# bcgsc/btl_bloomfilter

Hardware: AMD Instinct MI355X
Metric: Mk-mers/s insert+query, k=31 h=4, 64 GiB filter (higher is better)
Workload: dtype u64

## Files before the change

btl_bloomfilter_amd/build.py:

```python
import os
import subprocess
import sys
from concurrent.futures import ThreadPoolExecutor

HERE = os.path.dirname(os.path.abspath(__file__))
CSRC = os.path.join(HERE, "csrc")
TAG = os.environ.get("BTLBF_BUILD_TAG", "")
OBJ = os.path.join(HERE, "_build" + ("_" + TAG if TAG else ""))
LIB = os.path.join(HERE, "libbtlbf%s.so" % ("_" + TAG if TAG else ""))
HEADERS = ["internal.hpp", "mibf_plan.hpp", "mibf_zip.hpp", "mibf_classify_core.hpp", "host_internal.hpp", "host_partition.hpp", "device_utils.hpp", "seq_core.hpp", "partition_core.hpp",
           os.path.join("..", "..", "include", "btlbf.h")]
HOST_UNITS = ["capi", "host_io", "host_seq", "host_query", "host_partition", "host_aux", "host_mibf", "host_mibf_probs",
              "host_mibf_fastx", "fastx"]
KERNEL_UNITS = ["seq_kernels", "aux_kernels", "split_query_kernels", "partition_kernels", "mibf_kernels", "mibf_classify_kernels",
                "mibf_classify_pair_kernels", "mibf_stream_kernels"]
UNITS = [(u, u + ".cpp", []) for u in HOST_UNITS] + [(u, u + ".hip", []) for u in KERNEL_UNITS]
UNITS += [("part_hash_h%d" % h, "part_hash_inst.hip", ["-DBTLBF_PART_H=%d" % h]) for h in range(1, 9)]
FLAGS = ["--offload-arch=gfx950", "-O3", "-std=c++17", "-fPIC", "-Wall", "-Wno-unused-function"]


def _newest_header():
    return max(os.path.getmtime(os.path.join(CSRC, h)) for h in HEADERS + ["../build.py"])


def _extra_flags():
# ... 51 lines not shown
```

btl_bloomfilter_amd/csrc/host_partition.cpp:

```cpp
#include "../../include/btlbf.h"
#include "internal.hpp"
#include "host_internal.hpp"
#include "host_partition.hpp"

#include <algorithm>
#include <cmath>
#include <cstdlib>
#include <cstring>
#include <vector>

using namespace btlbf;

namespace {

static constexpr uint64_t kFailCap = 4ull << 20;
static constexpr uint64_t kFailTableSlots = 2 * kFailCap;
static constexpr uint64_t kFreshSpillCap = 16ull << 20;

uint32_t chunks_for(double mean_entries, uint32_t tail_chunks, uint32_t epc = kChunk)
{
	const double m = mean_entries + 8.0 * std::sqrt(mean_entries + 1.0) + 32.0;
	return (uint32_t)std::min<double>(4.0e9, std::ceil(m / (double)epc)) + tail_chunks;
}

unsigned ceil_log2(uint64_t x)
{
	unsigned b = 0;
	while ((1ull << b) < x)
		++b;
	return b;
}

bool plan_segments(uint64_t mloc, PartPlan& pl, uint32_t unit_shift = 3)
{
	const uint32_t small = 16 + unit_shift;
	pl.counting = unit_shift == 0;
	pl.seg_shift = small;
	if (((mloc + (1ull << small) - 1) >> small) > 512ull * 1024)
// ... 56 lines not shown
		for (int j = 1; j < pl.n_levels; ++j) {
			pl.lv[j].regions = split_slices(bins_g, r_in, cus);
			r_in = pl.lv[j].regions;
			bins_g *= pl.lv[j].P;
		}
	}
	return true;
}

bool packed_enabled()
{
	const char* e = getenv("BTLBF_PACKED");
	return !(e && e[0] == '0');
}

void plan_caps(PartPlan& pl, double entries, int first_level)
{
	pl.bytes_total = 0;
	for (int j = first_level; j < pl.n_levels; ++j) {
		PartLevel& l = pl.lv[j];
		const double useful = j == pl.n_levels - 1 ? (double)std::min<uint64_t>(pl.n_seg, l.bins) : (double)l.bins;
		l.packed = j >= 1 && j == pl.n_levels - 1 && !pl.counting && part_packs(l.P, l.shift) && packed_enabled();
		l.cap = chunks_for(entries / (useful * l.regions), 1, part_epc(l.packed));
		l.alloc_bins = l.bins;
		if (j >= 1 && pl.group_bins) {
			l.alloc_bins = pl.group_bins;
			for (int i = 1; i <= j; ++i)
				l.alloc_bins *= pl.lv[i].P;
		}
		l.cnt_bytes = ((uint64_t)l.alloc_bins * l.regions * 4 + 255) / 256 * 256;
		l.ent_bytes = (uint64_t)l.alloc_bins * l.regions * l.cap * (kChunk * 4);
		pl.bytes_total += l.cnt_bytes + l.ent_bytes;
	}
}

uint8_t* carve_levels(PartPlan& pl, uint8_t* p, int first_level)
{
	for (int j = first_level; j < pl.n_levels; ++j) {
		pl.lv[j].cnt = reinterpret_cast<uint32_t*>(p);
		p += pl.lv[j].cnt_bytes;
		pl.lv[j].ent = reinterpret_cast<uint32_t*>(p);
		p += pl.lv[j].ent_bytes;
	}
	return p;
}

unsigned cu_count(int device)
{
	int cus = 256;
	(void)hipDeviceGetAttribute(&cus, hipDeviceAttributeMultiprocessorCount, device);
	return (unsigned)cus;
}

uint64_t tiles_for_caps(uint64_t tiles, uint32_t regions)
{
	return regions ? (tiles + regions - 1) / regions * regions : tiles;
}

double probes_per_tile(const btlbf_filter* f, const PartTiling& tl)
{
	return tl.windows_per_tile * f->hp.h + 1.0;
}

PartSide part_side(const btlbf_filter* f, const PartPlan* pl = nullptr)
{
	PartSide sd;
	memset(&sd, 0, sizeof sd);
	sd.pos_base = f->mod.shard_lo;
	sd.counting = f->kind == BTLBF_COUNTING8;
	sd.threshold = f->thr;
	if (pl) {
		sd.late_buf = pl->late_buf;
		sd.late_cap = pl->late_cap;
		sd.bin_wseg = pl->lv[0].wseg;
		sd.bin_magic = pl->lv[0].wseg ? (uint32_t)(((1ull << 32) + pl->lv[0].wseg - 1) / pl->lv[0].wseg) : 0;
		sd.bin_seg_shift = pl->seg_shift;
		sd.bin_width = pl->lv[0].wseg << pl->seg_shift;
	}
	return sd;
}

int run_levels(btlbf_filter* f, PartPlan& pl, PartIn in0, const PartSide& sd, int query, hipStream_t s,
               uint32_t bin_offset = 0, uint32_t n_bins0 = 0)
{
	const int exact = sd.counting && !query;
	if (f->lazy_zero && !(sd.fresh && !query))
		return fail(BTLBF_EINVAL, "internal error: partition passes on a lazily cleared array");
	const int prof_split = query ? BTLBF_PROF_QUERY_SPLIT : BTLBF_PROF_INSERT_SPLIT;
	const int prof_apply = query ? BTLBF_PROF_QUERY_TEST : BTLBF_PROF_INSERT_APPLY;
	if (n_bins0 == 0)
		n_bins0 = pl.lv[0].bins - bin_offset;
	const uint32_t group = pl.group(n_bins0);
	for (uint32_t b0 = 0; b0 < n_bins0; b0 += group) {
		PartIn in = in0;
		uint32_t first_in = b0, abs_first = bin_offset + b0, n_in = std::min(group, n_bins0 - b0);
		uint32_t in_shift = pl.lv[0].shift;
		for (int j = 1; j < pl.n_levels; ++j) {
			ProfSpan ps(f, prof_split, s);
			HIP_TRY(launch_part_split(f->d_data, in, first_in, abs_first, n_in, pl.lv[j].out(), pl.lv[j].shift,
			                          in_shift, sd, query, exact, s));
			in = pl.lv[j].in();
			first_in = 0;
			abs_first *= pl.lv[j].P;
			n_in *= pl.lv[j].P;
			in_shift = pl.lv[j].shift;
		}
		const uint64_t seg_first = abs_first;
		if (seg_first >= pl.n_seg)
			break;
		const uint64_t n_seg = std::min<uint64_t>(n_in, pl.n_seg - seg_first);
		ProfSpan ps(f, prof_apply, s);
		HIP_TRY(launch_part_apply(f->d_data, f->local_bytes, pl.seg_shift, seg_first, n_seg, in, sd, query, s));
	}
	return BTLBF_OK;
}

constexpr double kAutoInsertRatio = 0.0095;
constexpr double kWideSplitProbes = 1.6e10;

}

namespace btlbf {

PartTail part_tail(uint64_t budget)
{
	PartTail t;
	const bool full = budget >= (2ull << 30);
// ... 88 lines not shown
	if (level0)
		pl = *level0;
	else if (!plan_level0(f, pl, call_probes(f, base.len)))
		return pp;
	PartLevel& l0 = pl.lv[0];
	l0.regions = cu_count(f->device);
	if (!plan_splits(pl, l0.regions, cu_count(f->device)) || !part_hash_fits(f->hp, l0.P))
		return pp;
	pp.tiling = part_tiling(f->hp, l0.P, base.layout, base.len);
	const uint64_t budget = scratch_budget(f);
	pp.tail = part_tail(budget);
	pl.late_cap = budget >= (2ull << 30) ? part_late_cap() : 0;
	const uint64_t late_bytes = (uint64_t)l0.regions * 2 * pl.late_cap * sizeof(uint32_t);
	const uint64_t extra_bytes = ((pp.tail.bytes + 255) / 256) * 256 + late_bytes;
	const double ppt = probes_per_tile(f, pp.tiling) * ((double)f->mod.shard_len / (double)f->mod.size);
	uint64_t tiles = pp.tiling.n_tiles;
	for (int iter = 0; iter < 64; ++iter) {
		plan_caps(pl, (double)tiles_for_caps(tiles, l0.regions) * ppt, 0);
		pl.bytes_total += extra_bytes;
		if (pl.bytes_total <= budget || tiles <= 1)
			break;
		const double ratio = (double)budget / (double)pl.bytes_total;
		const uint64_t nt = (uint64_t)((double)tiles * ratio * 0.95);
		tiles = nt >= tiles ? tiles - 1 : (nt ? nt : 1);
	}
	if (pl.bytes_total > budget)
		return pp;
	if (mode == BTLBF_INSERT_AUTO && tiles < pp.tiling.n_tiles && (double)tiles * ppt < auto_ratio * (double)f->local_bytes)
		return pp;
	pl.tiles_per_batch = tiles;
	if (!f->part.grow(pl.bytes_total, f->device))
		return pp;
	pp.extra = carve_levels(pl, static_cast<uint8_t*>(f->part.p), 0);
	pl.late_buf = pl.late_cap ? reinterpret_cast<uint32_t*>(pp.extra + ((pp.tail.bytes + 255) / 256) * 256) : nullptr;
	pp.ok = true;
	return pp;
}

struct RoutePlan {
	uint32_t n_windows = 1;
	uint32_t shards_per_window = 1;
	uint32_t window_shift = 0;
	uint32_t bins = 1024;
	uint32_t shift0 = 0;
	uint32_t bins_per_shard = 0;
	uint32_t regions = 0;
	uint32_t cap = 0;
	uint64_t ent_bytes_per_shard = 0, cnt_bytes_per_shard = 0;
// ... 23 lines not shown
	rp.bins = rp.window_shift - 9 <= 32 && rp.shards_per_window <= 512 ? 512 : 1024;
	if (const char* e = getenv("BTLBF_ROUTE_BINS")) {
		const unsigned b = (unsigned)atoi(e);
		if (b >= rp.shards_per_window && b <= 1024 && !(b & (b - 1)))
			rp.bins = b;
	}
	const unsigned lw = rp.window_shift, lb = ceil_log2(rp.bins);
	const unsigned seg_min = f->kind == BTLBF_COUNTING8 ? 16 : 19;
	if (lw < lb + seg_min || lw - lb > 32 || rp.bins < rp.shards_per_window)
		return fail(BTLBF_EINVAL, "routing supports global filters of at least 2^29 bits (2^26 counters)");
	rp.shift0 = lw - lb;
	rp.bins_per_shard = rp.bins / rp.shards_per_window;
	rp.regions = cu_count(f->device);
	const PartTiling tl = part_tiling(f->hp, rp.bins, lay, len);
	const double entries = (double)tiles_for_caps(tl.n_tiles, rp.regions) * probes_per_tile(f, tl) / rp.n_windows;
	rp.cap = chunks_for(entries / ((double)rp.bins * rp.regions), 1);
	rp.ent_bytes_per_shard = (uint64_t)rp.bins_per_shard * rp.regions * rp.cap * (kChunk * 4);
	rp.cnt_bytes_per_shard = (uint64_t)rp.bins_per_shard * rp.regions * 4;
	return BTLBF_OK;
}

int owner_plan(btlbf_filter* f, const RoutePlan& rp, const LayoutParams& lay, uint64_t plan_len, unsigned n_blocks,
               unsigned n_shards, PartPlan& pl)
{
	if (!plan_segments(f->mod.shard_len, pl, f->kind == BTLBF_COUNTING8 ? 0 : 3))
		return fail(BTLBF_EINVAL, "shard too large for the partitioned pipeline");
	pl.lv[0].bins = rp.bins_per_shard;
	pl.lv[0].shift = rp.shift0;
	pl.lv[0].regions = rp.regions * n_blocks;
	if (pl.lv[0].shift < pl.seg_shift || !plan_splits(pl, pl.lv[0].regions, cu_count(f->device)))
		return fail(BTLBF_EINVAL, "unsupported shard geometry");
// ... 69 lines not shown
		return false;
	if (f->insert_mode == BTLBF_INSERT_PARTITIONED)
		return true;
	return worth_sweep(f, local_probes(f, len), kAutoInsertRatio);
}

int partitioned_insert(btlbf_filter* f, const SeqArgs& base, hipStream_t s, bool* done)
{
	*done = false;
	PartPrep pp = part_prepare(f, base, f->insert_mode, kAutoInsertRatio);
	if (!pp.ok)
		return BTLBF_OK;
	PartPlan& pl = pp.pl;
	const uint64_t total_tiles = pp.tiling.n_tiles;
	for (uint64_t t0 = 0; t0 < total_tiles; t0 += pl.tiles_per_batch) {
		SeqArgs a = base;
		a.first_tile = t0;
		a.n_tiles = std::min<uint64_t>(pl.tiles_per_batch, total_tiles - t0);
		for (int attempt = 0; attempt < 2; ++attempt) {
			const bool fresh = f->lazy_zero;
			PartSide sd = part_side(f, &pl);
			if (fresh) {
				HIP_TRY(order_after_clear(f, s));
				sd.fresh = 1;
				sd.spill_count = reinterpret_cast<unsigned long long*>(pp.extra);
				sd.spill_list = reinterpret_cast<uint64_t*>(pp.extra + 256);
				sd.spill_cap = pp.tail.spill_cap;
				HIP_TRY(hipMemsetAsync(sd.spill_count, 0, 8, s));
			}
			{
				ProfSpan ps(f, BTLBF_PROF_INSERT_HASH, s);
				HIP_TRY(launch_part_hash(a, pl.lv[0].out(), pl.lv[0].shift, sd, 0, s));
			}
			if (int rc = run_levels(f, pl, pl.lv[0].in(), sd, 0, s))
				return rc;
			if (!fresh)
				break;
			f->lazy_zero = false;
			unsigned long long n_spill = 0;
			hipError_t e = hipMemcpyAsync(&n_spill, sd.spill_count, 8, hipMemcpyDeviceToHost, s);
			if (e == hipSuccess)
				e = hipStreamSynchronize(s);
			if (e == hipSuccess && n_spill <= pp.tail.spill_cap) {
				e = launch_spill(f->d_data, sd.spill_list, n_spill, f->mod.shard_lo, f->mod.shard_len, 0, part_side(f), s);
				if (e == hipSuccess)
					break;
			}
			if (e != hipSuccess) {
				f->lazy_zero = true;
// ... 15 lines not shown
		return BTLBF_OK;
	PartPlan& pl = pp.pl;
	const uint64_t total_tiles = pp.tiling.n_tiles;
	PartSide sd = part_side(f, &pl);
	sd.fail_count = reinterpret_cast<unsigned long long*>(pp.extra);
	sd.fail_list = reinterpret_cast<uint64_t*>(pp.extra + 256);
	sd.fail_cap = pp.tail.fail_cap;
	const int direct_op = direct_query_op(f);
	uint64_t* table = sd.fail_list + pp.tail.fail_cap;
	uint64_t* ctl = reinterpret_cast<uint64_t*>(pp.extra + 64);
	if (counts)
		HIP_TRY(hipMemsetAsync(counts, 0, 16, s));
	const uint64_t seq_tw = (uint64_t)seq_tile_windows();
	const uint64_t seq_tiles_all = (base.len + seq_tw - 1) / seq_tw;
	for (uint64_t t0 = 0; t0 < total_tiles; t0 += pl.tiles_per_batch) {
		SeqArgs a = base;
		a.first_tile = t0;
		a.n_tiles = std::min<uint64_t>(pl.tiles_per_batch, total_tiles - t0);
		a.hit_bits = hit_bits;
		a.valid_bits = valid_bits;
		a.counts = counts;
		HIP_TRY(hipMemsetAsync(sd.fail_count, 0, 8, s));
		{
			ProfSpan ps(f, BTLBF_PROF_QUERY_HASH, s);
			HIP_TRY(launch_part_hash(a, pl.lv[0].out(), pl.lv[0].shift, sd, 1, s));
		}
		if (int rc = run_levels(f, pl, pl.lv[0].in(), sd, 1, s))
			return rc;
		const uint64_t first = t0 * pp.tiling.tile_bytes / seq_tw;
		const uint64_t end_b = std::min<uint64_t>(base.len, (t0 + a.n_tiles) * (uint64_t)pp.tiling.tile_bytes);
		const uint64_t n = std::min<uint64_t>((end_b + seq_tw - 1) / seq_tw, seq_tiles_all) - first;
		ProfSpan ps(f, BTLBF_PROF_QUERY_RESOLVE, s);
		HIP_TRY(launch_failset_auto(sd.fail_list, sd.fail_count, pp.tail.fail_cap, table, pp.tail.table_slots, ctl, s));
		SeqArgs d = base;
		d.first_tile = first;
		d.n_tiles = n;
		d.hit_bits = hit_bits;
		d.valid_bits = nullptr;
		d.counts = nullptr;
		d.gate = ctl;
		d.gate_mode = GATE_REDO;
		REQUIRE_MATERIALIZED(f);
		HIP_TRY(launch_seq_op(direct_op, d, s));
		d.buckets = table;
		d.gate_mode = GATE_RESOLVE;
// ... 204 lines not shown
```

btl_bloomfilter_amd/csrc/host_partition.hpp:

```cpp
#pragma once
#include "host_internal.hpp"

namespace btlbf {

struct PartTail {
	uint64_t fail_cap, table_slots, spill_cap, bytes;
};
PartTail part_tail(uint64_t budget);

struct PartLevel {
	uint32_t bins = 0;
	uint32_t P = 0;
	uint32_t regions = 0;
	uint32_t cap = 0;
	uint32_t shift = 0;
	uint32_t wseg = 0;
	uint32_t alloc_bins = 0;
	uint32_t packed = 0;
	uint64_t cnt_bytes = 0, ent_bytes = 0;
	uint32_t* cnt = nullptr;
	uint32_t* ent = nullptr;
	PartOut out() const { return PartOut{P, regions, cap, packed, cnt, ent}; }
	PartIn in() const { return PartIn{1, alloc_bins, regions, cap, cnt, ent, packed}; }
};

struct PartPlan {
	uint32_t seg_shift = 19;
	uint64_t n_seg = 0;
	bool counting = false;
	uint32_t group_bins = 0;
	int n_levels = 0;
	PartLevel lv[3];
	uint64_t tiles_per_batch = 0;
	uint64_t bytes_total = 0;
	uint32_t* late_buf = nullptr;
	uint32_t late_cap = 0;
	uint32_t group(uint32_t n_bins0) const { return n_levels >= 2 && group_bins ? group_bins : n_bins0; }
};

constexpr double kAutoQueryRatio = 0.0165;

uint64_t scratch_budget(btlbf_filter* f);
double local_probes(const btlbf_filter* f, uint64_t len);
bool worth_sweep(const btlbf_filter* f, double probes, double ratio);
int direct_query_op(const btlbf_filter* f);
double call_probes(const btlbf_filter* f, uint64_t len);
bool plan_level0(const btlbf_filter* f, PartPlan& pl, double call_probes = 0);

int part_query(btlbf_filter* f, const SeqArgs& base, uint8_t* hit_bits, uint8_t* valid_bits, uint64_t* counts,
               hipStream_t s, bool* done, bool defer_hit_count, const PartPlan* level0);

// ... 2 lines not shown
```

btl_bloomfilter_amd/csrc/internal.hpp:

```cpp
#pragma once
#include <hip/hip_runtime.h>
#include <stdint.h>

#include "mibf_plan.hpp"

namespace btlbf {

static constexpr uint64_t kSeedA = 0x3c8bfbb395c60474ULL;
static constexpr uint64_t kSeedC = 0x3193c18562a02b4cULL;
static constexpr uint64_t kSeedG = 0x20323ed082572324ULL;
static constexpr uint64_t kSeedT = 0x295549f54be24456ULL;
static constexpr uint64_t kMultiSeed = 0x90b45d39fb6da1faULL;
static constexpr unsigned kMultiShift = 27;

static constexpr unsigned kCodeShift = 4u;
static constexpr unsigned kCodeOff = 0x70u;
static constexpr unsigned kNumCodes = 8u;
static constexpr unsigned kBaseValid = 1u;
static constexpr unsigned kBaseGood = 2u;

static constexpr uint32_t kChunk = 32;
static constexpr uint32_t kChunkShift = 5;
static constexpr uint32_t kPackChunk = 48;
static constexpr uint32_t kPackBits = 20;
// ... 140 lines not shown
	uint32_t late_cap;
	uint32_t* late_buf;
	uint32_t bin_wseg, bin_magic, bin_seg_shift, bin_width;
};
static inline uint32_t part_late_cap() { return 32768u; }

PartTiling part_tiling(const HashParams& hp, uint32_t p0, const LayoutParams& lay, uint64_t len);
bool part_supported(const HashParams& hp);
bool part_hash_fits(const HashParams& hp, uint32_t p0);
hipError_t launch_part_hash(const SeqArgs& a, const PartOut& out, uint32_t bin_shift, const PartSide& sd, int query,
                            hipStream_t s);
hipError_t launch_part_split(void* filter, const PartIn& in, uint32_t first_in, uint32_t abs_first, uint32_t n_in_bins,
                             const PartOut& out, uint32_t sub_shift, uint32_t in_shift, const PartSide& sd, int query,
                             int exact, hipStream_t s);
hipError_t launch_part_apply(void* filter, uint64_t local_bytes, uint32_t seg_shift, uint64_t seg_first, uint64_t n_seg,
                             const PartIn& in, const PartSide& sd, int query, hipStream_t s);
hipError_t launch_failset_build(const uint64_t* fail_list, uint64_t n, uint64_t* table, uint64_t mask, hipStream_t s);
enum { GATE_NONE = 0, GATE_RESOLVE = 1, GATE_REDO = 2 };
hipError_t launch_failset_auto(const uint64_t* fail_list, const unsigned long long* fail_count, uint64_t fail_cap,
                               uint64_t* table, uint64_t max_slots, uint64_t* ctl, hipStream_t s);
hipError_t launch_spill(void* filter, const uint64_t* pos, uint64_t n, uint64_t lo, uint64_t len, int test,
                        const PartSide& sd, hipStream_t s);
hipError_t launch_seq_op(int op, const SeqArgs& a, hipStream_t s);
hipError_t launch_hash_op(int op, void* filter, const ModParams& mod, uint32_t h, uint32_t threshold,
                          const uint64_t* hashes, uint64_t n, uint8_t* out, int serial, hipStream_t s,
                          const uint8_t* row_valid = nullptr);
hipError_t launch_kmer_rows(const uint8_t* kmers, uint64_t n, uint32_t k, uint32_t h, uint64_t kms, uint64_t* rows,
                            uint8_t* valid, hipStream_t s);
hipError_t launch_serial_seq_update(const SeqArgs& a, int op, const uint64_t* hashes,
                                    const uint8_t* valid_bits, uint8_t* out, hipStream_t s);
hipError_t launch_popcount(const void* data, uint64_t nbytes, int mode, uint32_t threshold,
// ... 123 lines not shown
```

btl_bloomfilter_amd/csrc/partition_kernels.hip:

```cpp
#include "partition_core.hpp"
#include <algorithm>

namespace btlbf {

typedef uint32_t v4u_t __attribute__((ext_vector_type(4)));
__device__ __forceinline__ uint4 nt_load4(const uint4* p)
{
	const v4u_t v = __builtin_nontemporal_load(reinterpret_cast<const v4u_t*>(p));
	return make_uint4(v.x, v.y, v.z, v.w);
}
__device__ __forceinline__ void nt_store4(uint4* p, const uint4& q)
{
	v4u_t v = {q.x, q.y, q.z, q.w};
	__builtin_nontemporal_store(v, reinterpret_cast<v4u_t*>(p));
}

__device__ __forceinline__ uint32_t part_in_region(const PartIn& in, uint32_t b, uint32_t r)
{
	return ((r / in.regions_per_block) * in.bins_per_block + b) * in.regions_per_block + r % in.regions_per_block;
}

template <bool QUERY, bool EXACT, bool PK>
__global__ __launch_bounds__(kPartThreads) void part_split_kernel(void* filter, const PartIn in, const PartOut out,
                                                                 const uint32_t slices, const uint32_t sub_shift,
// ... 73 lines not shown
			if (base1 >= n_vec)
				break;
			if (base1 + kPartThreads * kVec < n_vec)
				fetch(va, base1 + kPartThreads * kVec);
			round(vb, base1);
		}
	}
	if (PK)
		part_finish_pk<kPartThreads>(pl, out, bin0, g, ovf);
	else
		part_finish<kPartThreads>(pl, out, bin0, g, ovf);
}

static constexpr uint32_t kApplyMaxRegions = 1024;
static constexpr uint32_t kApplyFewRegions = 16;

enum ApplyMode : int {
	APPLY_BIT_OR = 0,
	APPLY_BIT_TEST = 1,
	APPLY_CNT_INC = 2,
	APPLY_CNT_TEST = 3
};

template <int MODE>
__device__ __forceinline__ void apply_entry(uint32_t* lds, uint32_t e, const PartSide& sd, uint64_t seg_base)
{
	if (MODE == APPLY_BIT_OR) {
		atomicOr(&lds[e >> 5], 1u << (e & 31));
	} else if (MODE == APPLY_BIT_TEST) {
		if (!((lds[e >> 5] >> (e & 31)) & 1u))
// ... 42 lines not shown
	} else {
		if (left > 0)
			apply_entry<MODE>(lds, q.x, sd, seg_base);
		if (left > 1)
			apply_entry<MODE>(lds, q.y, sd, seg_base);
		if (left > 2)
			apply_entry<MODE>(lds, q.z, sd, seg_base);
		if (left > 3)
			apply_entry<MODE>(lds, q.w, sd, seg_base);
	}
}

template <int MODE, int NT, bool PK>
__global__ __launch_bounds__(NT) void part_apply_kernel(uint8_t* filter, uint64_t local_bytes,
                                                        uint32_t seg_shift, uint32_t seg_first,
                                                        const PartIn in, const PartSide sd)
{
	constexpr bool QUERY = (MODE & 1) != 0;
	constexpr bool kNtEnt = !QUERY;
	constexpr uint32_t kUnitShift = MODE >= APPLY_CNT_INC ? 0 : 3;
	extern __shared__ __attribute__((aligned(16))) uint8_t dyn[];
	__shared__ uint32_t any;
	__shared__ uint32_t r_n[kApplyMaxRegions];
	__shared__ uint32_t r_reg[kApplyMaxRegions];
	const uint32_t tid = threadIdx.x;
	const uint32_t ibin = blockIdx.x;
	const uint32_t seg = seg_first + blockIdx.x;
	const uint32_t n_regions = in.blocks * in.regions_per_block;
	constexpr uint32_t kVecE = PK ? 6 : 4;
	const uint32_t cap_entries = in.cap * (PK ? kPackChunk : kChunk);
	const uint32_t cap_words = in.cap * kChunk;
	const bool tabled = n_regions <= kApplyMaxRegions;
	if (tid == 0)
		any = 0;
	__syncthreads();
	uint32_t mine = 0;
	for (uint32_t r = tid; r < n_regions; r += NT) {
		const uint32_t reg = part_in_region(in, ibin, r);
		uint32_t n = in.cnt[reg];
		if (n > cap_entries)
			n = cap_entries;
		mine |= n;
		if (tabled) {
			r_n[r] = n;
			r_reg[r] = reg;
		}
	}
	if (mine)
		any = 1;
	__syncthreads();
	if (!any && !(sd.fresh && !QUERY))
		return;
	const uint64_t seg_bytes = 1ull << (seg_shift - kUnitShift);
	const uint64_t byte0 = (uint64_t)seg * seg_bytes;
	const uint64_t seg_base = (uint64_t)seg << seg_shift;
	uint64_t nbytes = local_bytes - byte0;
	if (nbytes > seg_bytes)
		nbytes = seg_bytes;
	const uint32_t n_vec = (uint32_t)((nbytes + 15) / 16);
	uint4* lds4 = reinterpret_cast<uint4*>(dyn);
// ... 4 lines not shown
	uint4 q[kEntU];
#define BTLBF_SETTLE(r, i)                               \
	while ((r) < n_regions) {                            \
		const uint32_t nev__ = (r_n[(r)] + kVecE - 1) / kVecE; \
		if ((i) < nev__)                                 \
			break;                                       \
		(i) -= nev__;                                    \
		++(r);                                           \
	}
#define BTLBF_FETCH(dst, lft, u)                                                                               \
	do {                                                                                                       \
		lft = 0;                                                                                               \
		dst = make_uint4(0, 0, 0, 0);                                                                          \
		if (wr[u] < n_regions) {                                                                               \
			lft = r_n[wr[u]] - wi[u] * kVecE;                                                                  \
			dst = reinterpret_cast<const uint4*>(in.ent + (uint64_t)r_reg[wr[u]] * cap_words)[wi[u]];          \
		}                                                                                                      \
	} while (0)
	constexpr int kFewU = 3;
	const bool few = tabled && n_regions <= kApplyFewRegions;
	uint4 fq[kFewU];
	uint32_t fl[kFewU];
	uint32_t f_r = 0, f_off = 0;
	auto few_nvec = [&](uint32_t r) -> uint32_t {
		return ((uint32_t)__builtin_amdgcn_readfirstlane((int)r_n[r]) + kVecE - 1) / kVecE;
	};
	auto few_skip = [&]() {
		while (f_r < n_regions && f_off >= few_nvec(f_r)) {
			++f_r;
			f_off = 0;
		}
	};
	auto few_request = [&](uint4 (&d)[kFewU], uint32_t (&lf)[kFewU]) {
		const uint32_t n0 = (uint32_t)__builtin_amdgcn_readfirstlane((int)r_n[f_r]), nv0 = (n0 + kVecE - 1) / kVecE;
		const uint32_t reg0 = (uint32_t)__builtin_amdgcn_readfirstlane((int)r_reg[f_r]);
		const bool two = f_r + 1 < n_regions;
		const uint32_t n1 = two ? (uint32_t)__builtin_amdgcn_readfirstlane((int)r_n[two ? f_r + 1 : f_r]) : 0u, nv1 = (n1 + kVecE - 1) / kVecE;
		const uint32_t reg1 = two ? (uint32_t)__builtin_amdgcn_readfirstlane((int)r_reg[two ? f_r + 1 : f_r]) : reg0;
		const uint4* src0 = reinterpret_cast<const uint4*>(in.ent + (uint64_t)reg0 * cap_words);
		const uint4* src1 = reinterpret_cast<const uint4*>(in.ent + (uint64_t)reg1 * cap_words);
#pragma unroll
		for (int u = 0; u < kFewU; ++u) {
			const uint32_t v = f_off + (uint32_t)u * NT + tid;
			lf[u] = 0;
			d[u] = make_uint4(0, 0, 0, 0);
			if (v < nv0) {
				d[u] = kNtEnt ? nt_load4(src0 + v) : src0[v];
				lf[u] = n0 - v * kVecE;
			} else if (v - nv0 < nv1) {
				d[u] = kNtEnt ? nt_load4(src1 + (v - nv0)) : src1[v - nv0];
				lf[u] = n1 - (v - nv0) * kVecE;
			}
		}
		const uint32_t end = f_off + (uint32_t)(kFewU * NT);
		if (end <= nv0) {
// ... 67 lines not shown
				wi[u] += kEntU * NT;
				BTLBF_SETTLE(wr[u], wi[u])
				BTLBF_FETCH(nq[u], nleft[u], u);
			}
#pragma unroll
			for (int u = 0; u < kEntU; ++u) {
				apply_vec<MODE, PK>(lds, q[u], left[u], sd, seg_base);
				q[u] = nq[u];
				left[u] = nleft[u];
			}
		}
#undef BTLBF_SETTLE
#undef BTLBF_FETCH
	} else {
		for (uint32_t r = 0; r < n_regions; ++r) {
			const uint32_t reg = part_in_region(in, ibin, r);
			uint32_t n = in.cnt[reg];
			if (n > cap_entries)
				n = cap_entries;
			const uint32_t* e1 = in.ent + (uint64_t)reg * cap_words;
			if (PK) {
				for (uint32_t i = tid; i < (n + 2) / 3; i += NT) {
					uint32_t e3[3];
					part_unpack3(e1[2 * i], e1[2 * i + 1], e3);
					apply_entry<MODE>(lds, e3[0], sd, seg_base);
					apply_entry<MODE>(lds, e3[1], sd, seg_base);
					apply_entry<MODE>(lds, e3[2], sd, seg_base);
				}
				continue;
			}
			for (uint32_t i = tid; i < n; i += NT)
				apply_entry<MODE>(lds, e1[i], sd, seg_base);
		}
	}
	if (QUERY)
// ... 168 lines not shown
	                   abs_first - first_in, sd);
}

template <int NT>
static auto apply_kernel(int mode, bool packed) -> decltype(&part_apply_kernel<APPLY_BIT_OR, NT, false>)
{
	switch (mode) {
	case APPLY_BIT_OR: return packed ? &part_apply_kernel<APPLY_BIT_OR, NT, true> : &part_apply_kernel<APPLY_BIT_OR, NT, false>;
	case APPLY_BIT_TEST: return packed ? &part_apply_kernel<APPLY_BIT_TEST, NT, true> : &part_apply_kernel<APPLY_BIT_TEST, NT, false>;
	case APPLY_CNT_INC: return &part_apply_kernel<APPLY_CNT_INC, NT, false>;
	default: return &part_apply_kernel<APPLY_CNT_TEST, NT, false>;
	}
}

hipError_t launch_part_apply(void* filter, uint64_t local_bytes, uint32_t seg_shift, uint64_t seg_first, uint64_t n_seg,
                             const PartIn& in, const PartSide& sd, int query, hipStream_t s)
{
	if (n_seg == 0)
		return hipSuccess;
	if (in.packed && (sd.counting || seg_shift > kPackBits))
		return hipErrorInvalidValue;
	const int mode = (sd.counting ? APPLY_CNT_INC : APPLY_BIT_OR) + (query ? 1 : 0);
	const size_t dyn = (size_t)1 << (seg_shift - (sd.counting ? 0 : 3));
	const bool wide = dyn > 64 * 1024;
	return part_launch(wide ? apply_kernel<1024>(mode, in.packed) : apply_kernel<512>(mode, in.packed), dim3((unsigned)n_seg),
	                   dim3(wide ? 1024 : 512), dyn, s, static_cast<uint8_t*>(filter), local_bytes, seg_shift, (uint32_t)seg_first,
	                   in, sd);
}

__device__ __forceinline__ void failset_insert(unsigned long long* table, uint64_t mask, unsigned long long key)
{
	uint64_t slot = mix64(key) & mask;
	for (;;) {
		const unsigned long long prev = atomicCAS(&table[slot], 0ull, key);
		if (prev == 0ull || prev == key)
			break;
		slot = (slot + 1) & mask;
	}
}
__global__ __launch_bounds__(256) void failset_build_kernel(const uint64_t* list, uint64_t n,
                                                           unsigned long long* table, uint64_t mask)
{
// ... 90 lines not shown
```

Baseline: 61730.

## Carry level-0 split batches into a single final apply pass over the filter

When the partition scratch budget forces the input to be split into several tile batches, earlier batches are now hashed and split into per-batch carried buckets instead of each running a full apply pass. The final batch's apply kernel then reads both the current and carried buckets, so each filter segment is loaded into LDS and written back once per call instead of once per batch. A planner in a new header picks the number of carried batches and their sizes to fit the budget. The cost is more scratch bookkeeping, extra split launches, and an apply kernel that addresses regions through a shared arena base with 32-bit chunk offsets.

```diff
diff --git a/btl_bloomfilter_amd/build.py b/btl_bloomfilter_amd/build.py
--- a/btl_bloomfilter_amd/build.py
+++ b/btl_bloomfilter_amd/build.py
@@ -8,7 +8,7 @@
 TAG = os.environ.get("BTLBF_BUILD_TAG", "")
 OBJ = os.path.join(HERE, "_build" + ("_" + TAG if TAG else ""))
 LIB = os.path.join(HERE, "libbtlbf%s.so" % ("_" + TAG if TAG else ""))
-HEADERS = ["internal.hpp", "mibf_plan.hpp", "mibf_zip.hpp", "mibf_classify_core.hpp", "host_internal.hpp", "host_partition.hpp", "device_utils.hpp", "seq_core.hpp", "partition_core.hpp",
+HEADERS = ["internal.hpp", "mibf_plan.hpp", "part_plan.hpp", "mibf_zip.hpp", "mibf_classify_core.hpp", "host_internal.hpp", "host_partition.hpp", "device_utils.hpp", "seq_core.hpp", "partition_core.hpp",
            os.path.join("..", "..", "include", "btlbf.h")]
 HOST_UNITS = ["capi", "host_io", "host_seq", "host_query", "host_partition", "host_aux", "host_mibf", "host_mibf_probs",
               "host_mibf_fastx", "fastx"]
diff --git a/btl_bloomfilter_amd/csrc/host_partition.cpp b/btl_bloomfilter_amd/csrc/host_partition.cpp
--- a/btl_bloomfilter_amd/csrc/host_partition.cpp
+++ b/btl_bloomfilter_amd/csrc/host_partition.cpp
@@ -2,9 +2,11 @@
 #include "internal.hpp"
 #include "host_internal.hpp"
 #include "host_partition.hpp"
+#include "part_plan.hpp"
 
 #include <algorithm>
 #include <cmath>
+#include <cstdio>
 #include <cstdlib>
 #include <cstring>
 #include <vector>
@@ -17,11 +19,7 @@
 static constexpr uint64_t kFailTableSlots = 2 * kFailCap;
 static constexpr uint64_t kFreshSpillCap = 16ull << 20;
 
-uint32_t chunks_for(double mean_entries, uint32_t tail_chunks, uint32_t epc = kChunk)
-{
-	const double m = mean_entries + 8.0 * std::sqrt(mean_entries + 1.0) + 32.0;
-	return (uint32_t)std::min<double>(4.0e9, std::ceil(m / (double)epc)) + tail_chunks;
-}
+static_assert(kPlanChunkBytes == kChunk * 4, "part_plan.hpp counts chunks of kChunk words");
 
 unsigned ceil_log2(uint64_t x)
 {
@@ -108,6 +106,19 @@
 	return !(e && e[0] == '0');
 }
 
+bool carry_enabled()
+{
+	const char* e = getenv("BTLBF_CARRY");
+	return !(e && e[0] == '0');
+}
+
+uint32_t carry_forced()
+{
+	const char* e = getenv("BTLBF_CARRY_FORCE");
+	const int v = e ? atoi(e) : 0;
+	return v >= 1 && v <= (int)kCarryMaxBatches ? (uint32_t)v : 0;
+}
+
 void plan_caps(PartPlan& pl, double entries, int first_level)
 {
 	pl.bytes_total = 0;
@@ -115,15 +126,16 @@
 		PartLevel& l = pl.lv[j];
 		const double useful = j == pl.n_levels - 1 ? (double)std::min<uint64_t>(pl.n_seg, l.bins) : (double)l.bins;
 		l.packed = j >= 1 && j == pl.n_levels - 1 && !pl.counting && part_packs(l.P, l.shift) && packed_enabled();
-		l.cap = chunks_for(entries / (useful * l.regions), 1, part_epc(l.packed));
 		l.alloc_bins = l.bins;
 		if (j >= 1 && pl.group_bins) {
 			l.alloc_bins = pl.group_bins;
 			for (int i = 1; i <= j; ++i)
 				l.alloc_bins *= pl.lv[i].P;
 		}
-		l.cnt_bytes = ((uint64_t)l.alloc_bins * l.regions * 4 + 255) / 256 * 256;
-		l.ent_bytes = (uint64_t)l.alloc_bins * l.regions * l.cap * (kChunk * 4);
+		const LevelBytes lb = level_bytes(entries, useful, l.alloc_bins, l.regions, part_epc(l.packed));
+		l.cap = lb.cap;
+		l.cnt_bytes = lb.cnt_bytes;
+		l.ent_bytes = lb.ent_bytes;
 		pl.bytes_total += l.cnt_bytes + l.ent_bytes;
 	}
 }
@@ -144,11 +156,6 @@
 	int cus = 256;
 	(void)hipDeviceGetAttribute(&cus, hipDeviceAttributeMultiprocessorCount, device);
 	return (unsigned)cus;
-}
-
-uint64_t tiles_for_caps(uint64_t tiles, uint32_t regions)
-{
-	return regions ? (tiles + regions - 1) / regions * regions : tiles;
 }
 
 double probes_per_tile(const btlbf_filter* f, const PartTiling& tl)
@@ -175,7 +182,7 @@
 }
 
 int run_levels(btlbf_filter* f, PartPlan& pl, PartIn in0, const PartSide& sd, int query, hipStream_t s,
-               uint32_t bin_offset = 0, uint32_t n_bins0 = 0)
+               uint32_t bin_offset = 0, uint32_t n_bins0 = 0, const PartIn* carried = nullptr)
 {
 	const int exact = sd.counting && !query;
 	if (f->lazy_zero && !(sd.fresh && !query))
@@ -204,7 +211,43 @@
 			break;
 		const uint64_t n_seg = std::min<uint64_t>(n_in, pl.n_seg - seg_first);
 		ProfSpan ps(f, prof_apply, s);
-		HIP_TRY(launch_part_apply(f->d_data, f->local_bytes, pl.seg_shift, seg_first, n_seg, in, sd, query, s));
+		HIP_TRY(launch_part_apply(f->d_data, f->local_bytes, pl.seg_shift, seg_first, n_seg, in, sd, query, s, f->part.p,
+		                          carried));
+	}
+	return BTLBF_OK;
+}
+
+struct PartUnit {
+	uint64_t first = 0, n = 0;
+};
+PartUnit part_unit(const PartPlan& pl, uint64_t total_tiles, uint64_t t0)
+{
+	if (pl.carry_k)
+		return PartUnit{0, total_tiles};
+	return PartUnit{t0, std::min<uint64_t>(pl.tiles_per_batch, total_tiles - t0)};
+}
+
+int run_unit(btlbf_filter* f, PartPlan& pl, SeqArgs a, const PartUnit& u, const PartSide& sd, int query, hipStream_t s)
+{
+	const int exact = sd.counting && !query;
+	const uint32_t k = pl.carry_k;
+	const PartIn carried = pl.carry_in();
+	for (uint32_t j = 0; j <= k; ++j) {
+		a.first_tile = u.first + j * pl.carry_tiles;
+		a.n_tiles = j < k ? pl.carry_tiles : u.n - k * pl.carry_tiles;
+		{
+			ProfSpan ps(f, query ? BTLBF_PROF_QUERY_HASH : BTLBF_PROF_INSERT_HASH, s);
+			HIP_TRY(launch_part_hash(a, pl.lv[0].out(), pl.lv[0].shift, sd, query, s));
+		}
+		if (j < k) {
+			if (f->lazy_zero && !(sd.fresh && !query))
+				return fail(BTLBF_EINVAL, "internal error: partition passes on a lazily cleared array");
+			ProfSpan ps(f, query ? BTLBF_PROF_QUERY_SPLIT : BTLBF_PROF_INSERT_SPLIT, s);
+			HIP_TRY(launch_part_split(f->d_data, pl.lv[0].in(), 0, 0, pl.lv[0].bins, pl.carry_out(j), pl.carry.shift,
+			                          pl.lv[0].shift, sd, query, exact, s));
+		} else if (int rc = run_levels(f, pl, pl.lv[0].in(), sd, query, s, 0, 0, k ? &carried : nullptr)) {
+			return rc;
+		}
 	}
 	return BTLBF_OK;
 }
@@ -323,24 +366,71 @@
 	const uint64_t late_bytes = (uint64_t)l0.regions * 2 * pl.late_cap * sizeof(uint32_t);
 	const uint64_t extra_bytes = ((pp.tail.bytes + 255) / 256) * 256 + late_bytes;
 	const double ppt = probes_per_tile(f, pp.tiling) * ((double)f->mod.shard_len / (double)f->mod.size);
-	uint64_t tiles = pp.tiling.n_tiles;
-	for (int iter = 0; iter < 64; ++iter) {
-		plan_caps(pl, (double)tiles_for_caps(tiles, l0.regions) * ppt, 0);
+	auto batch_bytes = [&](uint64_t t) {
+		plan_caps(pl, (double)tiles_for_caps(t, l0.regions) * ppt, 0);
 		pl.bytes_total += extra_bytes;
-		if (pl.bytes_total <= budget || tiles <= 1)
-			break;
-		const double ratio = (double)budget / (double)pl.bytes_total;
-		const uint64_t nt = (uint64_t)((double)tiles * ratio * 0.95);
-		tiles = nt >= tiles ? tiles - 1 : (nt ? nt : 1);
-	}
-	if (pl.bytes_total > budget)
+		return pl.bytes_total;
+	};
+	const uint64_t tiles = batch_tiles_for_budget(pp.tiling.n_tiles, budget, batch_bytes);
+	if (tiles == 0)
 		return pp;
-	if (mode == BTLBF_INSERT_AUTO && tiles < pp.tiling.n_tiles && (double)tiles * ppt < auto_ratio * (double)f->local_bytes)
+	batch_bytes(tiles);
+	const uint32_t forced = carry_enabled() ? carry_forced() : 0;
+	if ((tiles < pp.tiling.n_tiles || forced) && pl.n_levels == 2 && pl.group_bins && carry_enabled()) {
+		CarryGeom g;
+		g.n_tiles = pp.tiling.n_tiles;
+		g.probes_per_tile = ppt;
+		g.regions0 = l0.regions;
+		g.bins0 = l0.bins;
+		g.bins1 = pl.lv[1].bins;
+		g.useful1 = std::min<uint64_t>(pl.n_seg, pl.lv[1].bins);
+		g.group_bins1 = pl.lv[1].alloc_bins;
+		g.regions_group = pl.lv[1].regions;
+		g.regions_carry = split_slices(l0.bins, l0.regions, cu_count(f->device));
+		g.epc1 = part_epc(pl.lv[1].packed);
+		g.extra_bytes = extra_bytes;
+		const CarryPlan cp = forced ? plan_forced(g, budget, forced) : plan_call(g, budget);
+		if (cp.K) {
+			auto take = [](PartLevel& l, const LevelBytes& b) {
+				l.cap = b.cap;
+				l.cnt_bytes = b.cnt_bytes;
+				l.ent_bytes = b.ent_bytes;
+			};
+			take(l0, cp.l0);
+			take(pl.lv[1], cp.group);
+			pl.carry = pl.lv[1];
+			pl.carry.regions = g.regions_carry;
+			pl.carry.alloc_bins = pl.carry.bins;
+			pl.carry.cap = cp.block.cap;
+			pl.carry.cnt_bytes = cp.carry_cnt_bytes;
+			pl.carry.ent_bytes = cp.K * cp.block.ent_bytes;
+			pl.carry_k = cp.K;
+			pl.carry_tiles = cp.tiles_carried;
+			pl.bytes_total = cp.bytes_total;
+		}
+	}
+	if (mode == BTLBF_INSERT_AUTO && !pl.carry_k && tiles < pp.tiling.n_tiles &&
+	    (double)tiles * ppt < auto_ratio * (double)f->local_bytes)
 		return pp;
-	pl.tiles_per_batch = tiles;
+	pl.tiles_per_batch = pl.carry_k ? pp.tiling.n_tiles : tiles;
 	if (!f->part.grow(pl.bytes_total, f->device))
 		return pp;
+	if (getenv("BTLBF_PLAN_LOG"))
+		fprintf(stderr,
+		        "btlbf plan: budget %llu tiles %llu carried batches %u of %llu tiles (independent batches of %llu) scratch %llu "
+		        "level0 %llu group %llu carried %llu caps %u %u %u\n",
+		        (unsigned long long)budget, (unsigned long long)pp.tiling.n_tiles, pl.carry_k, (unsigned long long)pl.carry_tiles,
+		        (unsigned long long)pl.tiles_per_batch, (unsigned long long)pl.bytes_total,
+		        (unsigned long long)(l0.cnt_bytes + l0.ent_bytes),
+		        (unsigned long long)(pl.n_levels >= 2 ? pl.lv[1].cnt_bytes + pl.lv[1].ent_bytes : 0),
+		        (unsigned long long)(pl.carry_k ? pl.carry.cnt_bytes + pl.carry.ent_bytes : 0), l0.cap,
+		        pl.n_levels >= 2 ? pl.lv[1].cap : 0, pl.carry_k ? pl.carry.cap : 0);
 	pp.extra = carve_levels(pl, static_cast<uint8_t*>(f->part.p), 0);
+	if (pl.carry_k) {
+		pl.carry.cnt = reinterpret_cast<uint32_t*>(pp.extra);
+		pl.carry.ent = reinterpret_cast<uint32_t*>(pp.extra + pl.carry.cnt_bytes);
+		pp.extra += pl.carry.cnt_bytes + pl.carry.ent_bytes;
+	}
 	pl.late_buf = pl.late_cap ? reinterpret_cast<uint32_t*>(pp.extra + ((pp.tail.bytes + 255) / 256) * 256) : nullptr;
 	pp.ok = true;
 	return pp;
@@ -394,7 +484,7 @@
 	rp.regions = cu_count(f->device);
 	const PartTiling tl = part_tiling(f->hp, rp.bins, lay, len);
 	const double entries = (double)tiles_for_caps(tl.n_tiles, rp.regions) * probes_per_tile(f, tl) / rp.n_windows;
-	rp.cap = chunks_for(entries / ((double)rp.bins * rp.regions), 1);
+	rp.cap = chunks_for(entries / ((double)rp.bins * rp.regions), 1, kChunk);
 	rp.ent_bytes_per_shard = (uint64_t)rp.bins_per_shard * rp.regions * rp.cap * (kChunk * 4);
 	rp.cnt_bytes_per_shard = (uint64_t)rp.bins_per_shard * rp.regions * 4;
 	return BTLBF_OK;
@@ -494,9 +584,7 @@
 	PartPlan& pl = pp.pl;
 	const uint64_t total_tiles = pp.tiling.n_tiles;
 	for (uint64_t t0 = 0; t0 < total_tiles; t0 += pl.tiles_per_batch) {
-		SeqArgs a = base;
-		a.first_tile = t0;
-		a.n_tiles = std::min<uint64_t>(pl.tiles_per_batch, total_tiles - t0);
+		const PartUnit u = part_unit(pl, total_tiles, t0);
 		for (int attempt = 0; attempt < 2; ++attempt) {
 			const bool fresh = f->lazy_zero;
 			PartSide sd = part_side(f, &pl);
@@ -508,11 +596,7 @@
 				sd.spill_cap = pp.tail.spill_cap;
 				HIP_TRY(hipMemsetAsync(sd.spill_count, 0, 8, s));
 			}
-			{
-				ProfSpan ps(f, BTLBF_PROF_INSERT_HASH, s);
-				HIP_TRY(launch_part_hash(a, pl.lv[0].out(), pl.lv[0].shift, sd, 0, s));
-			}
-			if (int rc = run_levels(f, pl, pl.lv[0].in(), sd, 0, s))
+			if (int rc = run_unit(f, pl, base, u, sd, 0, s))
 				return rc;
 			if (!fresh)
 				break;
@@ -558,21 +642,16 @@
 	const uint64_t seq_tw = (uint64_t)seq_tile_windows();
 	const uint64_t seq_tiles_all = (base.len + seq_tw - 1) / seq_tw;
 	for (uint64_t t0 = 0; t0 < total_tiles; t0 += pl.tiles_per_batch) {
+		const PartUnit u = part_unit(pl, total_tiles, t0);
 		SeqArgs a = base;
-		a.first_tile = t0;
-		a.n_tiles = std::min<uint64_t>(pl.tiles_per_batch, total_tiles - t0);
 		a.hit_bits = hit_bits;
 		a.valid_bits = valid_bits;
 		a.counts = counts;
 		HIP_TRY(hipMemsetAsync(sd.fail_count, 0, 8, s));
-		{
-			ProfSpan ps(f, BTLBF_PROF_QUERY_HASH, s);
-			HIP_TRY(launch_part_hash(a, pl.lv[0].out(), pl.lv[0].shift, sd, 1, s));
-		}
-		if (int rc = run_levels(f, pl, pl.lv[0].in(), sd, 1, s))
+		if (int rc = run_unit(f, pl, a, u, sd, 1, s))
 			return rc;
-		const uint64_t first = t0 * pp.tiling.tile_bytes / seq_tw;
-		const uint64_t end_b = std::min<uint64_t>(base.len, (t0 + a.n_tiles) * (uint64_t)pp.tiling.tile_bytes);
+		const uint64_t first = u.first * pp.tiling.tile_bytes / seq_tw;
+		const uint64_t end_b = std::min<uint64_t>(base.len, (u.first + u.n) * (uint64_t)pp.tiling.tile_bytes);
 		const uint64_t n = std::min<uint64_t>((end_b + seq_tw - 1) / seq_tw, seq_tiles_all) - first;
 		ProfSpan ps(f, BTLBF_PROF_QUERY_RESOLVE, s);
 		HIP_TRY(launch_failset_auto(sd.fail_list, sd.fail_count, pp.tail.fail_cap, table, pp.tail.table_slots, ctl, s));
diff --git a/btl_bloomfilter_amd/csrc/host_partition.hpp b/btl_bloomfilter_amd/csrc/host_partition.hpp
--- a/btl_bloomfilter_amd/csrc/host_partition.hpp
+++ b/btl_bloomfilter_amd/csrc/host_partition.hpp
@@ -35,6 +35,16 @@
 	uint64_t bytes_total = 0;
 	uint32_t* late_buf = nullptr;
 	uint32_t late_cap = 0;
+	uint32_t carry_k = 0;
+	uint64_t carry_tiles = 0;
+	PartLevel carry;
+	PartOut carry_out(uint32_t j) const
+	{
+		const uint64_t regs = (uint64_t)carry.bins * carry.regions;
+		return PartOut{carry.P, carry.regions, carry.cap, carry.packed, carry.cnt + j * regs,
+		               carry.ent + j * regs * carry.cap * kChunk};
+	}
+	PartIn carry_in() const { return PartIn{carry_k, carry.bins, carry.regions, carry.cap, carry.cnt, carry.ent, carry.packed}; }
 	uint32_t group(uint32_t n_bins0) const { return n_levels >= 2 && group_bins ? group_bins : n_bins0; }
 };
 
diff --git a/btl_bloomfilter_amd/csrc/internal.hpp b/btl_bloomfilter_amd/csrc/internal.hpp
--- a/btl_bloomfilter_amd/csrc/internal.hpp
+++ b/btl_bloomfilter_amd/csrc/internal.hpp
@@ -178,7 +178,8 @@
                              const PartOut& out, uint32_t sub_shift, uint32_t in_shift, const PartSide& sd, int query,
                              int exact, hipStream_t s);
 hipError_t launch_part_apply(void* filter, uint64_t local_bytes, uint32_t seg_shift, uint64_t seg_first, uint64_t n_seg,
-                             const PartIn& in, const PartSide& sd, int query, hipStream_t s);
+                             const PartIn& in, const PartSide& sd, int query, hipStream_t s, const void* arena = nullptr,
+                             const PartIn* carried = nullptr);
 hipError_t launch_failset_build(const uint64_t* fail_list, uint64_t n, uint64_t* table, uint64_t mask, hipStream_t s);
 enum { GATE_NONE = 0, GATE_RESOLVE = 1, GATE_REDO = 2 };
 hipError_t launch_failset_auto(const uint64_t* fail_list, const unsigned long long* fail_count, uint64_t fail_cap,
diff --git a/btl_bloomfilter_amd/csrc/part_plan.hpp b/btl_bloomfilter_amd/csrc/part_plan.hpp
--- /dev/null
+++ b/btl_bloomfilter_amd/csrc/part_plan.hpp
@@ -0,0 +1,163 @@
+#pragma once
+#include <stdint.h>
+
+#include <algorithm>
+#include <cmath>
+
+namespace btlbf {
+
+static constexpr uint32_t kPlanChunkBytes = 128;
+static constexpr uint32_t kCarryMaxBatches = 4;
+static constexpr uint32_t kCarryMaxRegions = 16;
+static constexpr uint32_t kCarryMaxTabled = 1024;
+static constexpr uint32_t kCarryGrid = 4096;
+
+inline uint32_t chunks_for(double mean_entries, uint32_t tail_chunks, uint32_t epc)
+{
+	const double m = mean_entries + 8.0 * std::sqrt(mean_entries + 1.0) + 32.0;
+	return (uint32_t)std::min<double>(4.0e9, std::ceil(m / (double)epc)) + tail_chunks;
+}
+
+inline uint64_t tiles_for_caps(uint64_t tiles, uint32_t regions)
+{
+	return regions ? (tiles + regions - 1) / regions * regions : tiles;
+}
+
+struct LevelBytes {
+	uint32_t cap = 0;
+	uint64_t cnt_bytes = 0, ent_bytes = 0;
+	uint64_t bytes() const { return cnt_bytes + ent_bytes; }
+};
+inline LevelBytes level_bytes(double entries, double useful_bins, uint64_t alloc_bins, uint32_t regions, uint32_t epc)
+{
+	LevelBytes b;
+	b.cap = chunks_for(entries / (useful_bins * regions), 1, epc);
+	b.cnt_bytes = (alloc_bins * regions * 4 + 255) / 256 * 256;
+	b.ent_bytes = alloc_bins * regions * b.cap * kPlanChunkBytes;
+	return b;
+}
+
+template <class F>
+inline uint64_t batch_tiles_for_budget(uint64_t n_tiles, uint64_t budget, F bytes_of)
+{
+	uint64_t tiles = n_tiles;
+	for (int iter = 0; iter < 64; ++iter) {
+		const uint64_t bytes = bytes_of(tiles);
+		if (bytes <= budget || tiles <= 1)
+			break;
+		const double ratio = (double)budget / (double)bytes;
+		const uint64_t nt = (uint64_t)((double)tiles * ratio * 0.95);
+		tiles = nt >= tiles ? tiles - 1 : (nt ? nt : 1);
+	}
+	return bytes_of(tiles) <= budget ? tiles : 0;
+}
+
+struct CarryGeom {
+	uint64_t n_tiles = 0;
+	double probes_per_tile = 0;
+	uint32_t regions0 = 0;
+	uint32_t bins0 = 0;
+	uint64_t bins1 = 0;
+	uint64_t useful1 = 0;
+	uint64_t group_bins1 = 0;
+	uint32_t regions_group = 0;
+	uint32_t regions_carry = 0;
+	uint32_t epc1 = 32;
+	uint64_t extra_bytes = 0;
+};
+
+struct CarryPlan {
+	uint32_t K = 0;
+	uint64_t tiles_per_batch = 0;
+	uint64_t tiles_carried = 0;
+	LevelBytes l0, group, block;
+	uint64_t carry_cnt_bytes = 0;
+	uint64_t bytes_total = 0;
+	uint64_t tiles_final(uint64_t n_tiles) const { return n_tiles - K * tiles_carried; }
+	uint64_t phase_first(uint32_t j) const { return (uint64_t)j * tiles_carried; }
+	uint64_t phase_tiles(uint32_t j, uint64_t n_tiles) const { return j < K ? tiles_carried : tiles_final(n_tiles); }
+	uint64_t phase_bytes(uint32_t j, const CarryGeom& g) const
+	{
+		const uint64_t blocks = std::min<uint64_t>(j + 1, K);
+		return g.extra_bytes + l0.bytes() + carry_cnt_bytes + blocks * block.ent_bytes + (j >= K ? group.bytes() : 0);
+	}
+};
+
+inline double carry_entries(const CarryGeom& g, uint64_t tiles)
+{
+	return (double)tiles_for_caps(tiles, g.regions0) * g.probes_per_tile;
+}
+
+inline uint64_t legacy_bytes(const CarryGeom& g, uint64_t tiles, LevelBytes* l0 = nullptr, LevelBytes* group = nullptr)
+{
+	const double e = carry_entries(g, tiles);
+	const LevelBytes a = level_bytes(e, (double)g.bins0, g.bins0, g.regions0, kPlanChunkBytes / 4);
+	const LevelBytes b = level_bytes(e, (double)g.useful1, g.group_bins1, g.regions_group, g.epc1);
+	if (l0)
+		*l0 = a;
+	if (group)
+		*group = b;
+	return a.bytes() + b.bytes() + g.extra_bytes;
+}
+
+inline CarryPlan carry_eval(const CarryGeom& g, uint32_t K, uint64_t tc)
+{
+	CarryPlan p;
+	p.K = K;
+	p.tiles_carried = tc;
+	const uint64_t tf = g.n_tiles - K * tc;
+	p.l0 = level_bytes(carry_entries(g, std::max(tc, tf)), (double)g.bins0, g.bins0, g.regions0, kPlanChunkBytes / 4);
+	p.group = level_bytes(carry_entries(g, tf), (double)g.useful1, g.group_bins1, g.regions_group, g.epc1);
+	p.block = level_bytes(carry_entries(g, tc), (double)g.useful1, g.bins1, g.regions_carry, g.epc1);
+	p.carry_cnt_bytes = (K * g.bins1 * g.regions_carry * 4 + 255) / 256 * 256;
+	p.bytes_total = p.phase_bytes(K, g);
+	return p;
+}
+
+inline bool carry_allowed(const CarryGeom& g, uint32_t K)
+{
+	const uint64_t most = g.regions_group <= kCarryMaxRegions ? kCarryMaxRegions : kCarryMaxTabled;
+	return g.regions_carry >= 1 && (uint64_t)g.regions_group + (uint64_t)K * g.regions_carry <= most && g.n_tiles >= K + 1;
+}
+
+inline uint64_t carry_candidate(const CarryGeom& g, uint32_t K, uint32_t i)
+{
+	const uint64_t hi = (g.n_tiles - 1) / K;
+	if (hi <= kCarryGrid)
+		return i >= 1 && i <= hi ? i : 0;
+	return (uint64_t)((unsigned __int128)hi * i / kCarryGrid);
+}
+
+inline CarryPlan plan_call(const CarryGeom& g, uint64_t budget, bool carry = true)
+{
+	CarryPlan legacy;
+	legacy.tiles_per_batch = batch_tiles_for_budget(g.n_tiles, budget, [&](uint64_t t) { return legacy_bytes(g, t); });
+	if (legacy.tiles_per_batch)
+		legacy.bytes_total = legacy_bytes(g, legacy.tiles_per_batch, &legacy.l0, &legacy.group);
+	if (!carry || legacy.tiles_per_batch == 0 || legacy.tiles_per_batch >= g.n_tiles)
+		return legacy;
+	for (uint32_t K = 1; K <= kCarryMaxBatches && carry_allowed(g, K); ++K) {
+		CarryPlan best;
+		for (uint32_t i = 1; i <= kCarryGrid; ++i) {
+			const uint64_t tc = carry_candidate(g, K, i);
+			if (tc == 0)
+				continue;
+			const CarryPlan p = carry_eval(g, K, tc);
+			if (p.bytes_total <= budget && (best.K == 0 || p.bytes_total < best.bytes_total))
+				best = p;
+		}
+		if (best.K)
+			return best;
+	}
+	return legacy;
+}
+
+inline CarryPlan plan_forced(const CarryGeom& g, uint64_t budget, uint32_t K)
+{
+	if (K < 1 || K > kCarryMaxBatches || !carry_allowed(g, K))
+		return CarryPlan();
+	const CarryPlan p = carry_eval(g, K, g.n_tiles / (K + 1));
+	return p.bytes_total <= budget ? p : CarryPlan();
+}
+
+}
diff --git a/btl_bloomfilter_amd/csrc/partition_kernels.hip b/btl_bloomfilter_amd/csrc/partition_kernels.hip
--- a/btl_bloomfilter_amd/csrc/partition_kernels.hip
+++ b/btl_bloomfilter_amd/csrc/partition_kernels.hip
@@ -1,4 +1,5 @@
 #include "partition_core.hpp"
+#include "part_plan.hpp"
 #include <algorithm>
 
 namespace btlbf {
@@ -111,6 +112,8 @@
 
 static constexpr uint32_t kApplyMaxRegions = 1024;
 static constexpr uint32_t kApplyFewRegions = 16;
+static_assert(kApplyFewRegions == kCarryMaxRegions && kApplyMaxRegions == kCarryMaxTabled,
+              "a carried plan keeps pass C on the walk the group buffer alone puts it on (part_plan.hpp)");
 
 enum ApplyMode : int {
 	APPLY_BIT_OR = 0,
@@ -183,7 +186,8 @@
 template <int MODE, int NT, bool PK>
 __global__ __launch_bounds__(NT) void part_apply_kernel(uint8_t* filter, uint64_t local_bytes,
                                                         uint32_t seg_shift, uint32_t seg_first,
-                                                        const PartIn in, const PartSide sd)
+                                                        const PartIn in, const PartSide sd,
+                                                        const uint32_t* arena, const PartIn cin)
 {
 	constexpr bool QUERY = (MODE & 1) != 0;
 	constexpr bool kNtEnt = !QUERY;
@@ -191,28 +195,36 @@
 	extern __shared__ __attribute__((aligned(16))) uint8_t dyn[];
 	__shared__ uint32_t any;
 	__shared__ uint32_t r_n[kApplyMaxRegions];
-	__shared__ uint32_t r_reg[kApplyMaxRegions];
+	__shared__ uint32_t r_base[kApplyMaxRegions];
 	const uint32_t tid = threadIdx.x;
 	const uint32_t ibin = blockIdx.x;
 	const uint32_t seg = seg_first + blockIdx.x;
-	const uint32_t n_regions = in.blocks * in.regions_per_block;
+	const uint32_t n_cur = in.blocks * in.regions_per_block;
+	const uint32_t n_regions = n_cur + cin.blocks * cin.regions_per_block;
 	constexpr uint32_t kVecE = PK ? 6 : 4;
-	const uint32_t cap_entries = in.cap * (PK ? kPackChunk : kChunk);
-	const uint32_t cap_words = in.cap * kChunk;
+	constexpr uint32_t kEpc = PK ? kPackChunk : kChunk;
+	const uint32_t cur0 = (uint32_t)((in.ent - arena) >> kChunkShift), car0 = (uint32_t)((cin.ent - arena) >> kChunkShift);
 	const bool tabled = n_regions <= kApplyMaxRegions;
+	auto region_at = [&](uint32_t r, uint32_t& n, uint32_t& base) {
+		const bool cur = r < n_cur;
+		const uint32_t reg = cur ? part_in_region(in, ibin, r) : part_in_region(cin, seg, r - n_cur);
+		const uint32_t cap = cur ? in.cap : cin.cap;
+		n = cur ? in.cnt[reg] : cin.cnt[reg];
+		if (n > cap * kEpc)
+			n = cap * kEpc;
+		base = (cur ? cur0 : car0) + reg * cap;
+	};
 	if (tid == 0)
 		any = 0;
 	__syncthreads();
 	uint32_t mine = 0;
 	for (uint32_t r = tid; r < n_regions; r += NT) {
-		const uint32_t reg = part_in_region(in, ibin, r);
-		uint32_t n = in.cnt[reg];
-		if (n > cap_entries)
-			n = cap_entries;
+		uint32_t n, cb;
+		region_at(r, n, cb);
 		mine |= n;
 		if (tabled) {
 			r_n[r] = n;
-			r_reg[r] = reg;
+			r_base[r] = cb;
 		}
 	}
 	if (mine)
@@ -247,7 +259,7 @@
 		dst = make_uint4(0, 0, 0, 0);                                                                          \
 		if (wr[u] < n_regions) {                                                                               \
 			lft = r_n[wr[u]] - wi[u] * kVecE;                                                                  \
-			dst = reinterpret_cast<const uint4*>(in.ent + (uint64_t)r_reg[wr[u]] * cap_words)[wi[u]];          \
+			dst = reinterpret_cast<const uint4*>(arena + (uint64_t)r_base[wr[u]] * kChunk)[wi[u]];             \
 		}                                                                                                      \
 	} while (0)
 	constexpr int kFewU = 3;
@@ -266,12 +278,12 @@
 	};
 	auto few_request = [&](uint4 (&d)[kFewU], uint32_t (&lf)[kFewU]) {
 		const uint32_t n0 = (uint32_t)__builtin_amdgcn_readfirstlane((int)r_n[f_r]), nv0 = (n0 + kVecE - 1) / kVecE;
-		const uint32_t reg0 = (uint32_t)__builtin_amdgcn_readfirstlane((int)r_reg[f_r]);
+		const uint32_t reg0 = (uint32_t)__builtin_amdgcn_readfirstlane((int)r_base[f_r]);
 		const bool two = f_r + 1 < n_regions;
 		const uint32_t n1 = two ? (uint32_t)__builtin_amdgcn_readfirstlane((int)r_n[two ? f_r + 1 : f_r]) : 0u, nv1 = (n1 + kVecE - 1) / kVecE;
-		const uint32_t reg1 = two ? (uint32_t)__builtin_amdgcn_readfirstlane((int)r_reg[two ? f_r + 1 : f_r]) : reg0;
-		const uint4* src0 = reinterpret_cast<const uint4*>(in.ent + (uint64_t)reg0 * cap_words);
-		const uint4* src1 = reinterpret_cast<const uint4*>(in.ent + (uint64_t)reg1 * cap_words);
+		const uint32_t reg1 = two ? (uint32_t)__builtin_amdgcn_readfirstlane((int)r_base[two ? f_r + 1 : f_r]) : reg0;
+		const uint4* src0 = reinterpret_cast<const uint4*>(arena + (uint64_t)reg0 * kChunk);
+		const uint4* src1 = reinterpret_cast<const uint4*>(arena + (uint64_t)reg1 * kChunk);
 #pragma unroll
 		for (int u = 0; u < kFewU; ++u) {
 			const uint32_t v = f_off + (uint32_t)u * NT + tid;
@@ -369,11 +381,9 @@
 #undef BTLBF_FETCH
 	} else {
 		for (uint32_t r = 0; r < n_regions; ++r) {
-			const uint32_t reg = part_in_region(in, ibin, r);
-			uint32_t n = in.cnt[reg];
-			if (n > cap_entries)
-				n = cap_entries;
-			const uint32_t* e1 = in.ent + (uint64_t)reg * cap_words;
+			uint32_t n, cb;
+			region_at(r, n, cb);
+			const uint32_t* e1 = arena + (uint64_t)cb * kChunk;
 			if (PK) {
 				for (uint32_t i = tid; i < (n + 2) / 3; i += NT) {
 					uint32_t e3[3];
@@ -572,18 +582,34 @@
 }
 
 hipError_t launch_part_apply(void* filter, uint64_t local_bytes, uint32_t seg_shift, uint64_t seg_first, uint64_t n_seg,
-                             const PartIn& in, const PartSide& sd, int query, hipStream_t s)
+                             const PartIn& in, const PartSide& sd, int query, hipStream_t s, const void* arena,
+                             const PartIn* carried)
 {
 	if (n_seg == 0)
 		return hipSuccess;
 	if (in.packed && (sd.counting || seg_shift > kPackBits))
 		return hipErrorInvalidValue;
+	PartIn cin{};
+	const uint32_t* base = in.ent;
+	if (carried && carried->blocks) {
+		cin = *carried;
+		base = static_cast<const uint32_t*>(arena);
+		const uint64_t chunk_b = kChunk * 4, off_in = (const uint8_t*)in.ent - (const uint8_t*)base,
+		               off_c = (const uint8_t*)cin.ent - (const uint8_t*)base;
+		if (!base || in.ent < base || cin.ent < base || off_in % chunk_b || off_c % chunk_b || cin.packed != in.packed ||
+		    seg_first + n_seg > cin.bins_per_block || cin.regions_per_block == 0)
+			return hipErrorInvalidValue;
+		const uint64_t end_in = off_in / chunk_b + (uint64_t)in.blocks * in.bins_per_block * in.regions_per_block * in.cap;
+		const uint64_t end_c = off_c / chunk_b + (uint64_t)cin.blocks * cin.bins_per_block * cin.regions_per_block * cin.cap;
+		if (std::max(end_in, end_c) > 0xffffffffull)
+			return hipErrorInvalidValue;
+	}
 	const int mode = (sd.counting ? APPLY_CNT_INC : APPLY_BIT_OR) + (query ? 1 : 0);
 	const size_t dyn = (size_t)1 << (seg_shift - (sd.counting ? 0 : 3));
 	const bool wide = dyn > 64 * 1024;
 	return part_launch(wide ? apply_kernel<1024>(mode, in.packed) : apply_kernel<512>(mode, in.packed), dim3((unsigned)n_seg),
 	                   dim3(wide ? 1024 : 512), dyn, s, static_cast<uint8_t*>(filter), local_bytes, seg_shift, (uint32_t)seg_first,
-	                   in, sd);
+	                   in, sd, base, cin);
 }
 
 __device__ __forceinline__ void failset_insert(unsigned long long* table, uint64_t mask, unsigned long long key)
```

Result: faster. 68300 (median of 6 runs) (+10.6%).
